# fxzjshm/simple-radio-telescope-backend

Hardware: AMD Instinct MI355X
Metric: baseband Msamples/sec/node + real-time ratio, J1644-4559 config at 1/2/4/8 MI355X (higher is better)
Workload: dtype fp32; 1 GPU; model=J1644-4559 coherent-dedispersion single-pulse pipeline, baseband_input_count=1073741824, nsamps_reserved=23494656, baseband_input_bits=2, spectrum_channel_count=2048, rfi=True, phase_table=False, fft_backend=native, parallelism=stream-sharded dp1, global_batch=1, seq_len=1073741824

## Files before the change

csrc/bind/module.cpp:

```cpp

#include <torch/extension.h>
#include <ATen/cuda/CUDAContext.h>
#include <c10/cuda/CUDAGuard.h>

#include <functional>
#include <vector>

#include "../engine/engine.h"
#include "../fft/native_fft.h"
#include "../include/srtb_kernels.h"

namespace {

using namespace srtb_hip;

hipStream_t cur_stream() {
  return at::cuda::getCurrentCUDAStream().stream();
}

void check(hipError_t e, const char* what) { check_hip(e, what); }

#define CHECK_CUDA(t) TORCH_CHECK((t).is_cuda(), #t " must be on GPU")
#define CHECK_CONTIG(t) TORCH_CHECK((t).is_contiguous(), #t " must be contiguous")

// ... 341 lines not shown
  CHECK_CONTIG(x);
  TORCH_CHECK(x.scalar_type() == torch::kComplexFloat);
  const size_t len = x.size(-1);
  const size_t batch = x.numel() / len;
  auto stream = cur_stream();
  NativeFft plan;
  plan.plan(len, batch, (int)sign, stream);
  auto out = torch::empty_like(x);
  if (plan.n_passes() == 1) {
    plan.exec(cptr(x), cptr(out), stream);
  } else {
    auto work = x.clone();
    plan.exec(cptr(work), cptr(out), stream);
  }
  check(hipStreamSynchronize(stream), "native_fft sync");
  return out;
}

torch::Tensor t_native_rfft(torch::Tensor x) {
  CHECK_CUDA(x);
  CHECK_CONTIG(x);
  TORCH_CHECK(x.scalar_type() == torch::kFloat32);
  const size_t n = x.numel();
  const size_t m = n / 2;
  auto stream = cur_stream();
  NativeFft plan;
  plan.plan(m, 1, -1, stream);
  auto z = torch::empty({(int64_t)m},
                        x.options().dtype(torch::kComplexFloat));
  auto packed = x.view({(int64_t)m, 2});
// ... 236 lines not shown
  m.def("sk_v1_mitigate", &t_sk_v1_mitigate, py::arg("wf"),
        py::arg("sk_threshold"), py::arg("normalize") = false);
  m.def("time_series", &t_time_series, py::arg("wf"), py::arg("flags"),
        py::arg("ts_count"));
  m.def("subtract_mean", &t_subtract_mean);
  m.def("count_signal", &t_count_signal);
  m.def("inclusive_scan", &t_inclusive_scan);
  m.def("boxcar", &t_boxcar);
  m.def("resample_power", &t_resample_power);
  m.def("normalize_by_mean", &t_normalize_by_mean);
  m.def("generate_pixmap", &t_generate_pixmap);
  m.def("running_mean", &t_running_mean);
  m.def("correlate", &t_correlate);
  m.def("native_fft", &t_native_fft, py::arg("x"), py::arg("sign"));
  m.def("native_rfft", &t_native_rfft, py::arg("x"));
  m.def("bench_fft", &t_bench_fft, py::arg("len"), py::arg("batch"),
        py::arg("sign"), py::arg("iters") = 20, py::arg("backend") = "native");
  m.def("bench_rfft", &t_bench_rfft, py::arg("n"), py::arg("iters") = 20,
        py::arg("backend") = "native");

  py::class_<PyEngine>(m, "PipelineEngine")
      .def(py::init<int64_t, int64_t, int64_t, double, double, double, double,
                    double, double, double, int64_t, int64_t,
                    std::vector<std::vector<int64_t>>, bool, bool, bool,
                    int64_t, int64_t, int64_t, bool>(),
           py::arg("n"), py::arg("nbits"), py::arg("channels"),
           py::arg("freq_low"), py::arg("bandwidth"), py::arg("sample_rate"),
           py::arg("dm"), py::arg("rfi_threshold") = 10.0,
           py::arg("sk_threshold") = 1.1, py::arg("snr_threshold") = 6.0,
           py::arg("max_boxcar") = 1024, py::arg("nsamps_reserved") = 0,
// ... 23 lines not shown
```

csrc/engine/engine.cpp:

```cpp
#include "engine.h"

#include <roctracer/roctx.h>

#include <cmath>
#include <cstdlib>
#include <cstring>
#include <stdexcept>

namespace srtb_hip {

namespace {
constexpr double kD = 4.148808e3;

struct RoctxRange {
  bool on;
  explicit RoctxRange(const char* name)
      : on([] {
          static const bool enabled = [] {
            const char* e = std::getenv("SRTB_ROCTX");
            return e && std::atoi(e) != 0;
          }();
          return enabled;
        }()) {
    if (on) roctxRangePush(name);
// ... 66 lines not shown
    if (n_boxcars_ > 0)
      check_hip(hipMalloc(&s.box_partials,
                          (size_t)n_boxcars_ * 2 * np * sizeof(double)),
                "box partials alloc");
    check_hip(hipMalloc(&s.mean_power, sizeof(double)), "mean alloc");
    check_hip(hipMalloc(&s.sums, 2 * sizeof(double)), "sums alloc");
    const int ncnt = 1 + 1 + n_boxcars_;
    check_hip(hipMalloc(&s.counters, ncnt * sizeof(unsigned)), "cnt alloc");
    check_hip(hipMalloc(&s.thresholds, (1 + n_boxcars_) * sizeof(float)),
              "thr alloc");
    check_hip(hipHostMalloc(&s.h_counters, ncnt * sizeof(unsigned)),
              "pinned cnt");
    check_hip(hipHostMalloc(&s.h_thresholds, (1 + n_boxcars_) * sizeof(float)),
              "pinned thr");
    fused_unpack_off_ = std::getenv("SRTB_NO_FUSED_UNPACK") != nullptr;
    const int be = cfg.fft_backend;
    native_fft_ = (be == 0 || be == 2) && NativeFft::supported(nc_);
    native_bwd_ = native_fft_ && NativeFft::supported(l_) &&
                  (be == 0 || l_ >= (1ull << 17));
    fuse_r2c_ = false;
    if (native_fft_) {
      s.nfwd.plan(nc_, 1, -1, s.stream);
      if (native_bwd_) {
        const char* b32 = std::getenv("SRTB_FFT_BWD32");
        if (b32 && std::atoi(b32) != 0)
          s.nbwd.plan(l_, s_, +1, s.stream, 5,
                      8);
        else
          s.nbwd.plan(l_, s_, +1, s.stream);
        const int wpr = s.nbwd.dif_sk_wgs_per_row();
// ... 78 lines not shown
  if (phase_table_) (void)hipFree(phase_table_);
  if (window_) (void)hipFree(window_);
  if (watfft_window_) (void)hipFree(watfft_window_);
}

void PipelineEngine::enqueue_chain(Slot& s, const uint8_t* dev_raw,
                                   const float* dev_samples, double dm,
                                   bool record_event) {
  hipStream_t st = s.stream;
  if (std::isnan(dm)) dm = cfg_.dm;
  const float2* table = phase_table_;
  if (table && dm != cfg_.dm)
    throw std::runtime_error("dm override requires use_phase_table=false");

  RoctxRange r_chain("srtb_block_chain");
  const float* fft_in = s.samples;
  const int in_bits = cfg_.baseband_input_bits;
  const bool fuse_unpack = dev_raw && native_fft_ && !fused_unpack_off_ &&
                           (in_bits == 1 || in_bits == 2 || in_bits == 4 ||
                            in_bits == 8 || in_bits == -8 ||
                            in_bits == 16 || in_bits == -16) &&
                           !window_ && slots_[0]->nfwd.first_pass_fusable();
  if (dev_raw && !fuse_unpack) {
    check_hip(unpack(dev_raw, s.samples, n_, cfg_.baseband_input_bits,
                     window_, st),
              "unpack");
  } else if (!dev_raw && native_fft_) {
    check_hip(hipMemcpyAsync(s.samples, dev_samples, n_ * sizeof(float),
                             hipMemcpyDeviceToDevice, st),
              "samples d2d");
  } else if (!dev_raw) {
    fft_in = dev_samples;
  }
  const bool fr2c = fuse_r2c_;
  if (native_fft_ && fr2c) {
    s.nfwd.exec(reinterpret_cast<float2*>(s.samples), s.spec, st,
                nullptr, cfg_.enable_rfi_s1 ? s.fwd_pw : nullptr,
                fuse_unpack ? dev_raw : nullptr, in_bits);
    if (cfg_.enable_rfi_s1)
      check_hip(r2c_mean_from_power(s.fwd_pw, fwd_pw_n_, s.spec, nc_,
                                    s.mean_power, st),
                "r2c mean");
  } else if (native_fft_) {
    s.nfwd.exec(reinterpret_cast<float2*>(s.samples), s.spec, st,
                nullptr, nullptr, fuse_unpack ? dev_raw : nullptr, in_bits);
    check_hip(r2c_post_process(
                  s.spec, s.spec, nc_,
                  cfg_.enable_rfi_s1 ? s.partials : nullptr,
                  cfg_.enable_rfi_s1 ? s.mean_power : nullptr, st),
              "r2c post");
  } else {
    s.plans.exec_r2c(const_cast<float*>(fft_in), s.spec);
    if (cfg_.enable_rfi_s1)
      check_hip(mean_power(s.spec, nc_, s.partials, s.mean_power, st),
                "meanp");
  }
  float2* wf;
  const bool fuse_into_bwd = native_bwd_ && s.nbwd.first_pass_fusable();
  if (fuse_into_bwd) {
    FftPreop pre;
    pre.mean_power = cfg_.enable_rfi_s1 ? s.mean_power : nullptr;
    pre.threshold = cfg_.rfi_threshold;
    pre.norm_coeff = norm_coeff_;
    pre.n_zap = cfg_.n_zap_ranges;
    for (int i = 0; i < cfg_.n_zap_ranges; ++i) pre.zap[i] = cfg_.zap_ranges[i];
    pre.f_min = f_min_;
    pre.f_c = f_c_;
    pre.df = df_;
    pre.dm = dm;
    pre.table = table;
    pre.r2c_m = fr2c ? nc_ : 0;
    s.nbwd.exec(s.spec, reinterpret_cast<float2*>(s.samples), st, &pre,
                watfft_window_ ? nullptr : s.sk_dif_partials, nullptr, 2,
                fr2c ? s.xbuf : nullptr);
    wf = reinterpret_cast<float2*>(s.samples);
  } else {
    check_hip(rfi_dedisperse_fused(
                  s.spec, nc_, cfg_.enable_rfi_s1 ? s.mean_power : nullptr,
                  cfg_.rfi_threshold, norm_coeff_, cfg_.zap_ranges,
                  cfg_.n_zap_ranges, f_min_, f_c_, df_, dm, table, st),
              "rfi+dedisp");
    if (native_bwd_) {
      s.nbwd.exec(s.spec, reinterpret_cast<float2*>(s.samples), st);
      wf = reinterpret_cast<float2*>(s.samples);
    } else {
      s.plans.exec_c2c_backward(s.spec);
// ... 37 lines not shown
    check_hip(boxcar_ladder(s.cumsum, ts_count_, boxcar_lengths_.data(),
                            n_boxcars_, s.box_partials, cfg_.snr_threshold,
                            s.thresholds + 1, s.counters + 2, st),
              "box ladder");
  }
  check_hip(hipMemcpyAsync(s.h_counters, s.counters, ncnt * sizeof(unsigned),
                           hipMemcpyDeviceToHost, st),
            "res d2h");
  check_hip(hipMemcpyAsync(s.h_thresholds, s.thresholds,
                           (1 + n_boxcars_) * sizeof(float),
                           hipMemcpyDeviceToHost, st),
            "thr d2h");
  if (record_event) {
    check_hip(hipEventRecord(s.done, st), "event record");
    s.busy = true;
  }
}

int PipelineEngine::submit(const void* host_bytes, size_t nbytes,
                           double dm_override) {
  if (nbytes != raw_bytes_) throw std::runtime_error("submit: wrong size");
  const int id = next_slot_;
  next_slot_ = (next_slot_ + 1) % n_slots_;
  Slot& s = *slots_[id];
  if (s.busy) {
    check_hip(hipEventSynchronize(s.done), "slot wait");
    s.busy = false;
  }
  const bool graph_ok = cfg_.use_hip_graph && std::isnan(dm_override);
  if (graph_ok && s.graph_exec && s.graph_host_src == host_bytes) {
// ... 118 lines not shown
```

csrc/engine/engine.h:

```cpp

#pragma once

#include <hip/hip_runtime.h>

#include <array>
#include <cstdint>
#include <memory>
#include <vector>

#include "../fft/fft_plans.h"
#include "../fft/native_fft.h"
#include "../include/srtb_kernels.h"

namespace srtb_hip {

struct EngineConfig {
  size_t baseband_input_count = 1ull << 28;
  int baseband_input_bits = 8;
  size_t spectrum_channel_count = 1ull << 15;
  double freq_low = 1000.0;
  double bandwidth = 500.0;
  double sample_rate = 1e9;
  double dm = 0.0;
  float rfi_threshold = 10.0f;
// ... 102 lines not shown
    double* box_partials = nullptr;
    double* mean_power = nullptr;
    double* sums = nullptr;
    unsigned* counters = nullptr;
    float* thresholds = nullptr;
    unsigned* h_counters = nullptr;
    float* h_thresholds = nullptr;
    FftPlanSet plans;
    NativeFft nfwd, nbwd;
    hipGraphExec_t graph_exec = nullptr;
    const void* graph_host_src = nullptr;
    int graph_pending = 0;
  };
  std::vector<std::unique_ptr<Slot>> slots_;
  int next_slot_ = 0;
};

}
```

csrc/fft/native_fft.h:

```cpp

#pragma once

#include <algorithm>
#include <cstdint>
#include <cstdlib>
#include <cmath>
#include <stdexcept>
#include <string>
#include <vector>

#include "../include/srtb_kernels.h"
#include "fft_plans.h"

namespace srtb_hip {

class NativeFft {
 public:
  static constexpr uint32_t kMaxPassLen = 4096;
  static int elems_per_wg() {
    const char* e = std::getenv("SRTB_FFT_ELEMS");
    int v = e ? std::atoi(e) : 4096;
    if (v < 512) v = 512;
    if (v > 8192) v = 8192;
    return v;
// ... 158 lines not shown
      p.dif.n_prefix = m - 1;
      for (int w = 0; w < m - 1; ++w) {
        p.dif.pf_bits[w] = ilog2z(f[w]);
        p.dif.pf_coef[w] = M[w + 1] / fn;
      }
      p.n_ffts = batch * (L / fn);
      p.tw_n = len_table(fn);
      passes_.push_back(p);
    }
  }

  int n_passes() const { return (int)passes_.size(); }

  bool first_pass_fusable() const {
    return !passes_.empty() && passes_[0].kind == PassKind::kCol;
  }

  int dif_sk_wgs_per_row() const {
    if (passes_.empty() || passes_.back().kind != PassKind::kDif) return 0;
    const Pass& p = passes_.back();
    const size_t per_row = (len_ / p.dif.n);
    const int F = dif_f(p);
    if (per_row % F != 0) return 0;
    return (int)(per_row / F);
  }

  void exec(const float2* in, float2* out, hipStream_t stream,
            const FftPreop* preop = nullptr,
            float2* dif_sk_partials = nullptr,
            const uint8_t* decode2_raw = nullptr, int decode_bits = 2,
// ... 174 lines not shown
```

csrc/include/srtb_kernels.h:

```cpp

#pragma once

#include <hip/hip_runtime.h>
#include <cstddef>
#include <cstdint>

namespace srtb_hip {

hipError_t unpack(const uint8_t* in, float* out, size_t out_count, int nbits,
                  const float* window, hipStream_t stream);

hipError_t unpack_interleaved_2pol(const int8_t* in, float* out0, float* out1,
                                   size_t count_per_pol, const float* window,
                                   hipStream_t stream);

hipError_t unpack_naocpsr_snap1(const int8_t* in, float* out0, float* out1,
                                size_t count_per_pol, const float* window,
                                hipStream_t stream);

hipError_t unpack_gznupsr_a1(const uint8_t* in, float* out0, float* out1,
                             float* out2, float* out3, int n_streams,
                             size_t count_per_stream, const float* window,
                             hipStream_t stream);

// ... 109 lines not shown
  double f_min = 0, f_c = 0, df = 0, dm = 0;
  const float2* table = nullptr;
  unsigned long long r2c_m = 0;
};

hipError_t r2c_mean_from_power(const float2* power_partials,
                               size_t n_partials, const float2* z0, size_t m,
                               double* out_mean, hipStream_t stream);

hipError_t fft_col_pass(const float2* in, float2* out, const FftPassDesc& d,
                        size_t n_ffts, int sign, const float2* tw_n,
                        const float2* tw_hi, const float2* tw_lo,
                        hipStream_t stream, const FftPreop* preop = nullptr,
                        const uint8_t* raw2 = nullptr, int raw_bits = 2);

struct DifFinalDesc {
  uint32_t n;
  unsigned long long out_c2;
  unsigned long long out_elem_coef;
  int n_prefix = 0;
  int pf_bits[4] = {0, 0, 0, 0};
  unsigned long long pf_coef[4] = {0, 0, 0, 0};
};
hipError_t fft_mid512_pass(const float2* in, float2* out,
                           const FftPassDesc& d, size_t n_ffts, int sign,
                           const float2* tw_n, hipStream_t stream);

hipError_t fft_dif_final(const float2* in, float2* out, const DifFinalDesc& d,
                         size_t n_ffts, int F, int sign, const float2* tw_n,
                         float2* sk_partials, hipStream_t stream);
// ... 35 lines not shown
```

csrc/kernels/common.h:

```cpp
#pragma once

#include <hip/hip_runtime.h>
#include <cstddef>
#include <cstdint>

namespace srtb_hip {

constexpr int kBlock = 256;
constexpr int kMaxBlocks = 4096;

inline dim3 grid_for(size_t n, int block = kBlock, int cap = kMaxBlocks) {
  size_t b = (n + block - 1) / block;
  if (b > static_cast<size_t>(cap)) b = cap;
  if (b == 0) b = 1;
  return dim3(static_cast<uint32_t>(b));
}

#define SRTB_CHECK_LAUNCH()                        \
  do {                                             \
    hipError_t err_ = hipGetLastError();           \
    if (err_ != hipSuccess) return err_;           \
  } while (0)


// ... 32 lines not shown

__device__ inline float2 srtb_dedisp_factor(size_t i, double f_min,
                                            double f_c, double df,
                                            double dm) {
  const double f = f_min + df * (double)i;
  const double r = (f - f_c) / f_c;
  const double k = (kDispersionConstantMHz * 1e6) * dm / f * (r * r);
  double k_int;
  const double k_frac = modf(k, &k_int);
  const float phi = (float)(-2.0 * M_PI * k_frac);
  float s, c;
  __sincosf(phi, &s, &c);
  return make_float2(c, s);
}

}
```

csrc/kernels/fft.hip:

```cpp

#include <cstdlib>
#include "common.h"
#include "../include/srtb_kernels.h"

namespace srtb_hip {

namespace {

__device__ inline float2 cmulf(float2 a, float2 b) {
  return make_float2(a.x * b.x - a.y * b.y, a.x * b.y + a.y * b.x);
}

}

struct FftPassDescDev {
  uint32_t n;
  int n_log2, f_log2;
  int d0_log2, d1_log2;
  unsigned long long in_c0, in_c1, in_c2;
  unsigned long long in_stride;
  unsigned long long out_c0, out_c1, out_c2;
  unsigned long long out_stride;
  unsigned long long tw_f0, tw_f1;
  unsigned long long tw_mask;
// ... 345 lines not shown
  if (k == 0) return make_float2(zk.x + zk.y, 0.0f);
  const float2 zm = zbase[m - k];
  const float2 zmc = make_float2(zm.x, -zm.y);
  const float2 even = make_float2(0.5f * (zk.x + zmc.x),
                                  0.5f * (zk.y + zmc.y));
  const float2 dif = make_float2(zk.x - zmc.x, zk.y - zmc.y);
  const float2 odd = make_float2(0.5f * dif.y, -0.5f * dif.x);
  const float phiw = (float)(-M_PI * (double)k / (double)m);
  float sw, cw;
  __sincosf(phiw, &sw, &cw);
  const float2 wo = make_float2(cw * odd.x - sw * odd.y,
                                cw * odd.y + sw * odd.x);
  return make_float2(even.x + wo.x, even.y + wo.y);
}

template <int N, bool TWIDDLE, int SIGN, bool PREOP, int DEC = 0>
__global__ void __launch_bounds__(256)
    k_fft_col(const float2* __restrict__ in, float2* __restrict__ out,
              FftPassDescDev d, unsigned long long n_ffts,
              const float2* __restrict__ tw_n,
              const float2* __restrict__ tw_hi,
              const float2* __restrict__ tw_lo, FftPreopDev pre,
              const uint8_t* __restrict__ raw2) {
  const unsigned long long id =
      (unsigned long long)xcd_swizzle(blockIdx.x, gridDim.x, d.tuning) *
          blockDim.x + threadIdx.x;
  if (id >= n_ffts) return;
  unsigned long long q0, q1, q2;
  digits(id, d, q0, q1, q2);
  const unsigned long long base = q0 * d.in_c0 + q1 * d.in_c1 + q2 * d.in_c2;
  float thr_mean = 0.f;
  if constexpr (PREOP) {
    if (pre.mean_power) thr_mean = pre.threshold * (float)(*pre.mean_power);
  }
  float2 v[N];
  const float2* __restrict__ colbase = in + base;
  const uint32_t stride32 = (uint32_t)d.in_stride;
#pragma unroll
  for (int i = 0; i < N; ++i) {
    const uint32_t off = (uint32_t)i * stride32;
    const unsigned long long flat = base + off;
    float2 x;
    if constexpr (DEC != 0) x = decN_load<DEC>(raw2, flat);
    else x = ld_stream(colbase + off, d.tuning);
    if constexpr (PREOP) {
      if (pre.r2c_m) x = r2c_combine_load(in, x, flat, pre.r2c_m);
      bool zap = pre.mean_power && (norm2(x) > thr_mean);
      for (int z = 0; z < pre.n_zap; ++z)
        zap |= (flat >= pre.zap[z].lo) & (flat <= pre.zap[z].hi);
      if (zap) {
        x = make_float2(0.f, 0.f);
      } else {
        if (pre.mean_power) {
          x.x *= pre.norm_coeff;
          x.y *= pre.norm_coeff;
        }
        x = cmulf(x, pre.table ? pre.table[flat]
                               : srtb_dedisp_factor(flat, pre.f_min, pre.f_c,
                                                    pre.df, pre.dm));
      }
    }
    v[col_sigma<N>(i)] = x;
  }
  col_fft<N, SIGN>(v, tw_n);
  float2* __restrict__ ocolbase = out + base;
#pragma unroll
  for (int k = 0; k < N; ++k) {
    float2 r = v[k];
    if constexpr (TWIDDLE) {
      const unsigned long long m_ =
          (q0 * d.tw_f0 * (unsigned long long)k) & d.tw_mask;
      r = cmulf(r, tw_eval(m_, d.tw_angle));
    }
    st_stream(ocolbase + (uint32_t)k * stride32, r, d.tuning);
  }
}


constexpr int col_sigma_inv64(int pos) {
  for (int i = 0; i < 64; ++i)
    if (col_sigma<64>(i) == pos) return i;
  return 0;
}

__device__ inline float2 shfl_xor1(float2 x) {
  return make_float2(__shfl_xor(x.x, 1, 64), __shfl_xor(x.y, 1, 64));
}

template <bool TWIDDLE, int SIGN, bool PREOP, int DEC = 0>
__global__ void __launch_bounds__(256)
    k_fft_col_pair64(const float2* __restrict__ in, float2* __restrict__ out,
                     FftPassDescDev d, unsigned long long n_ffts,
                     const float2* __restrict__ tw_n,
                     const float2* __restrict__ tw_hi,
                     const float2* __restrict__ tw_lo, FftPreopDev pre,
                     const uint8_t* __restrict__ raw2) {
  const unsigned long long tid =
      (unsigned long long)xcd_swizzle(blockIdx.x, gridDim.x, d.tuning) *
          blockDim.x + threadIdx.x;
  const unsigned long long id = tid >> 1;
  const int p = (int)(tid & 1);
  if (id >= n_ffts) return;
  unsigned long long q0, q1, q2;
  digits(id, d, q0, q1, q2);
  const unsigned long long base = q0 * d.in_c0 + q1 * d.in_c1 + q2 * d.in_c2;
  float thr_mean = 0.f;
  if constexpr (PREOP) {
    if (pre.mean_power) thr_mean = pre.threshold * (float)(*pre.mean_power);
  }
  float2 v[32];
  const float2* __restrict__ colbase = in + base;
  const uint32_t stride32 = (uint32_t)d.in_stride;
#pragma unroll
  for (int r = 0; r < 32; ++r) {
    const int i = p ? col_sigma_inv64(32 + r) : col_sigma_inv64(r);
    const uint32_t off = (uint32_t)i * stride32;
    float2 x;
    if constexpr (DEC != 0) x = decN_load<DEC>(raw2, base + off);
    else x = ld_stream(colbase + off, d.tuning);
    if constexpr (PREOP) {
      const unsigned long long flat = base + off;
      if (pre.r2c_m) x = r2c_combine_load(in, x, flat, pre.r2c_m);
      bool zap = pre.mean_power && (norm2(x) > thr_mean);
      for (int z = 0; z < pre.n_zap; ++z)
        zap |= (flat >= pre.zap[z].lo) & (flat <= pre.zap[z].hi);
      if (zap) {
        x = make_float2(0.f, 0.f);
      } else {
        if (pre.mean_power) {
          x.x *= pre.norm_coeff;
          x.y *= pre.norm_coeff;
        }
        x = cmulf(x, pre.table ? pre.table[flat]
                               : srtb_dedisp_factor(flat, pre.f_min, pre.f_c,
                                                    pre.df, pre.dm));
      }
    }
    v[r] = x;
  }
  col_stage<32, 4, 4, SIGN, 16>(v, tw_n);
  col_stage<32, 16, 4, SIGN, 4>(v, tw_n);
#pragma unroll
  for (int j = 0; j < 16; ++j) {
    const float2 ea = shfl_xor1(v[j]);
    const float2 eb = shfl_xor1(v[16 + j]);
    float2 a = p ? ea : v[j];
    float2 b = p ? eb : v[16 + j];
    float2 c = p ? v[j] : ea;
    float2 e = p ? v[16 + j] : eb;
    float2 w1, w2, w3;
// ... 17 lines not shown
      const unsigned long long m_ =
          (q0 * d.tw_f0 * (unsigned long long)k) & d.tw_mask;
      rr = cmulf(rr, tw_eval(m_, d.tw_angle));
    }
    st_stream(ocolbase + (uint32_t)k * stride32, rr, d.tuning);
  }
}


constexpr int col_sigma_inv32(int pos) {
  for (int i = 0; i < 32; ++i)
    if (col_sigma<32>(i) == pos) return i;
  return 0;
}

template <bool TWIDDLE, int SIGN, bool PREOP, int DEC = 0>
__global__ void __launch_bounds__(256)
    k_fft_col_pair32(const float2* __restrict__ in, float2* __restrict__ out,
                     FftPassDescDev d, unsigned long long n_ffts,
                     const float2* __restrict__ tw_n,
                     const float2* __restrict__ tw_hi,
                     const float2* __restrict__ tw_lo, FftPreopDev pre,
                     const uint8_t* __restrict__ raw2) {
  const unsigned long long tid =
      (unsigned long long)xcd_swizzle(blockIdx.x, gridDim.x, d.tuning) *
          blockDim.x + threadIdx.x;
  const unsigned long long id = tid >> 1;
  const int p = (int)(tid & 1);
  if (id >= n_ffts) return;
  unsigned long long q0, q1, q2;
  digits(id, d, q0, q1, q2);
  const unsigned long long base = q0 * d.in_c0 + q1 * d.in_c1 + q2 * d.in_c2;
  float thr_mean = 0.f;
  if constexpr (PREOP) {
    if (pre.mean_power) thr_mean = pre.threshold * (float)(*pre.mean_power);
  }
  float2 v[16];
  const float2* __restrict__ colbase = in + base;
  const uint32_t stride32 = (uint32_t)d.in_stride;
#pragma unroll
  for (int r = 0; r < 16; ++r) {
    const int i = p ? col_sigma_inv32(16 + r) : col_sigma_inv32(r);
    const uint32_t off = (uint32_t)i * stride32;
    float2 x;
    if constexpr (DEC != 0) x = decN_load<DEC>(raw2, base + off);
    else x = ld_stream(colbase + off, d.tuning);
    if constexpr (PREOP) {
      const unsigned long long flat = base + off;
      if (pre.r2c_m) x = r2c_combine_load(in, x, flat, pre.r2c_m);
      bool zap = pre.mean_power && (norm2(x) > thr_mean);
      for (int z = 0; z < pre.n_zap; ++z)
        zap |= (flat >= pre.zap[z].lo) & (flat <= pre.zap[z].hi);
      if (zap) {
        x = make_float2(0.f, 0.f);
      } else {
        if (pre.mean_power) {
          x.x *= pre.norm_coeff;
          x.y *= pre.norm_coeff;
        }
        x = cmulf(x, pre.table ? pre.table[flat]
                               : srtb_dedisp_factor(flat, pre.f_min, pre.f_c,
                                                    pre.df, pre.dm));
      }
    }
    v[r] = x;
  }
  col_stage<16, 4, 4, SIGN, 8>(v, tw_n);
  col_stage<16, 16, 4, SIGN, 2>(v, tw_n);
#pragma unroll
  for (int j = 0; j < 16; ++j) {
    const float2 other = shfl_xor1(v[j]);
    const float2 a = p ? other : v[j];
    const float2 b = p ? v[j] : other;
    const float2 w = (j == 0) ? make_float2(1.f, 0.f) : tw_n[j];
    const float2 y = cmulf(b, w);
    v[j] = p ? make_float2(a.x - y.x, a.y - y.y)
             : make_float2(a.x + y.x, a.y + y.y);
// ... 514 lines not shown
  } while (0)
  if (load_ffast) {
    if (store_ffast) DISPATCH2(true, true);
    else             DISPATCH2(true, false);
  } else {
    if (store_ffast) DISPATCH2(false, true);
    else             DISPATCH2(false, false);
  }
#undef DISPATCH2
#undef DISPATCH4
  SRTB_CHECK_LAUNCH();
  return hipSuccess;
}


hipError_t fft_col_pass(const float2* in, float2* out, const FftPassDesc& hd,
                        size_t n_ffts, int sign, const float2* tw_n,
                        const float2* tw_hi, const float2* tw_lo,
                        hipStream_t stream, const FftPreop* preop,
                        const uint8_t* raw2, int raw_bits) {
  if (raw2 && (preop || hd.tw_mod == 0)) return hipErrorInvalidValue;
  if (raw2 && raw_bits != 1 && raw_bits != 2 && raw_bits != 4 &&
      raw_bits != 8 && raw_bits != -8 && raw_bits != 16 && raw_bits != -16)
    return hipErrorInvalidValue;
  FftPreopDev pre{};
  if (preop) {
    pre.mean_power = preop->mean_power;
    pre.threshold = preop->threshold;
    pre.norm_coeff = preop->norm_coeff;
    pre.n_zap = preop->n_zap;
    for (int i = 0; i < preop->n_zap; ++i) pre.zap[i] = preop->zap[i];
    pre.f_min = preop->f_min;
    pre.f_c = preop->f_c;
    pre.df = preop->df;
    pre.dm = preop->dm;
    pre.table = preop->table;
    pre.r2c_m = preop->r2c_m;
  }
  FftPassDescDev d;
  d.n = hd.n;
  d.n_log2 = ilog2(hd.n);
  d.f_log2 = 0;
  d.d0_log2 = hd.d0 ? ilog2(hd.d0) : 48;
  d.d1_log2 = ilog2(hd.d1 ? hd.d1 : 1);
  d.in_c0 = hd.in_c0; d.in_c1 = hd.in_c1; d.in_c2 = hd.in_c2;
  d.in_stride = hd.in_stride;
  d.out_c0 = hd.out_c0; d.out_c1 = hd.out_c1; d.out_c2 = hd.out_c2;
  d.out_stride = hd.out_stride;
  d.tw_f0 = hd.tw_f0; d.tw_f1 = hd.tw_f1;
  d.tw_mask = hd.tw_mod ? hd.tw_mod - 1 : 0;
  d.tw_lo_bits = hd.tw_lo_bits;
  d.tw_angle = hd.tw_angle;
  d.tuning = fft_tuning();
// ... 11 lines not shown
#define COL_DISPATCH_D(N)                                                    \
  if (raw_bits == 1) { if (sign < 0) COL_LAUNCH_D(N, -1, 1);                 \
                       else COL_LAUNCH_D(N, 1, 1); }                         \
  else if (raw_bits == 2) { if (sign < 0) COL_LAUNCH_D(N, -1, 2);            \
                            else COL_LAUNCH_D(N, 1, 2); }                    \
  else if (raw_bits == 4) { if (sign < 0) COL_LAUNCH_D(N, -1, 4);            \
                            else COL_LAUNCH_D(N, 1, 4); }                    \
  else if (raw_bits == 8) { if (sign < 0) COL_LAUNCH_D(N, -1, 8);            \
                            else COL_LAUNCH_D(N, 1, 8); }                    \
  else if (raw_bits == -8) { if (sign < 0) COL_LAUNCH_D(N, -1, -8);          \
                             else COL_LAUNCH_D(N, 1, -8); }                  \
  else if (raw_bits == 16) { if (sign < 0) COL_LAUNCH_D(N, -1, 16);          \
                             else COL_LAUNCH_D(N, 1, 16); }                  \
  else { if (sign < 0) COL_LAUNCH_D(N, -1, -16);                             \
         else COL_LAUNCH_D(N, 1, -16); }
#define COL_DISPATCH(N)                                                      \
  case N:                                                                    \
    if (raw2) {                                                              \
      COL_DISPATCH_D(N)                                                      \
    } else if (twiddle) {                                                           \
      if (sign < 0) { if (preop) COL_LAUNCH(N, true, -1, true);              \
                      else COL_LAUNCH(N, true, -1, false); }                 \
      else          { if (preop) COL_LAUNCH(N, true, 1, true);               \
                      else COL_LAUNCH(N, true, 1, false); }                  \
    } else {                                                                 \
      if (sign < 0) { if (preop) COL_LAUNCH(N, false, -1, true);             \
                      else COL_LAUNCH(N, false, -1, false); }                \
      else          { if (preop) COL_LAUNCH(N, false, 1, true);              \
                      else COL_LAUNCH(N, false, 1, false); }                 \
    }                                                                        \
    break;
  const uint32_t grid2 = (uint32_t)((2 * n_ffts + 255) / 256);
#define COL_LAUNCH_P(TW, SG, PR)                                             \
// ... 6 lines not shown
                     tw_lo, pre, raw2)
#define COL_LAUNCH_P32(TW, SG, PR)                                           \
  hipLaunchKernelGGL((k_fft_col_pair32<TW, SG, PR>), dim3(grid2), dim3(256), \
                     0, stream, in, out, d, n_ffts, tw_n, tw_hi, tw_lo, pre, \
                     raw2)
#define COL_LAUNCH_P32D(SG, B)                                               \
  hipLaunchKernelGGL((k_fft_col_pair32<true, SG, false, B>), dim3(grid2),    \
                     dim3(256), 0, stream, in, out, d, n_ffts, tw_n, tw_hi,  \
                     tw_lo, pre, raw2)
  switch (hd.n) {
    COL_DISPATCH(2)
    COL_DISPATCH(4)
    COL_DISPATCH(8)
    COL_DISPATCH(16)
    case 32:
      if (use_pair32()) {
        if (raw2) {
          if (raw_bits == 1) { if (sign < 0) COL_LAUNCH_P32D(-1, 1);
                               else COL_LAUNCH_P32D(1, 1); }
          else if (raw_bits == 2) { if (sign < 0) COL_LAUNCH_P32D(-1, 2);
                                    else COL_LAUNCH_P32D(1, 2); }
          else if (raw_bits == 4) { if (sign < 0) COL_LAUNCH_P32D(-1, 4);
                                    else COL_LAUNCH_P32D(1, 4); }
          else if (raw_bits == 8) { if (sign < 0) COL_LAUNCH_P32D(-1, 8);
                                    else COL_LAUNCH_P32D(1, 8); }
          else if (raw_bits == -8) { if (sign < 0) COL_LAUNCH_P32D(-1, -8);
                                     else COL_LAUNCH_P32D(1, -8); }
          else if (raw_bits == 16) { if (sign < 0) COL_LAUNCH_P32D(-1, 16);
                                     else COL_LAUNCH_P32D(1, 16); }
          else { if (sign < 0) COL_LAUNCH_P32D(-1, -16);
// ... 18 lines not shown
        break;
      }
      if (twiddle) {
        if (sign < 0) { if (preop) COL_LAUNCH(32, true, -1, true);
                        else COL_LAUNCH(32, true, -1, false); }
        else          { if (preop) COL_LAUNCH(32, true, 1, true);
                        else COL_LAUNCH(32, true, 1, false); }
      } else {
        if (sign < 0) { if (preop) COL_LAUNCH(32, false, -1, true);
                        else COL_LAUNCH(32, false, -1, false); }
        else          { if (preop) COL_LAUNCH(32, false, 1, true);
                        else COL_LAUNCH(32, false, 1, false); }
      }
      break;
    case 64:
      if (raw2) {
        if (raw_bits == 1) { if (sign < 0) COL_LAUNCH_PD(-1, 1);
                             else COL_LAUNCH_PD(1, 1); }
        else if (raw_bits == 2) { if (sign < 0) COL_LAUNCH_PD(-1, 2);
                                  else COL_LAUNCH_PD(1, 2); }
        else if (raw_bits == 4) { if (sign < 0) COL_LAUNCH_PD(-1, 4);
                                  else COL_LAUNCH_PD(1, 4); }
        else if (raw_bits == 8) { if (sign < 0) COL_LAUNCH_PD(-1, 8);
                                  else COL_LAUNCH_PD(1, 8); }
        else if (raw_bits == -8) { if (sign < 0) COL_LAUNCH_PD(-1, -8);
                                   else COL_LAUNCH_PD(1, -8); }
        else if (raw_bits == 16) { if (sign < 0) COL_LAUNCH_PD(-1, 16);
                                   else COL_LAUNCH_PD(1, 16); }
        else { if (sign < 0) COL_LAUNCH_PD(-1, -16);
               else COL_LAUNCH_PD(1, -16); }
// ... 6 lines not shown
                        else COL_LAUNCH_P(true, 1, false); }
      } else {
        if (sign < 0) { if (preop) COL_LAUNCH_P(false, -1, true);
                        else COL_LAUNCH_P(false, -1, false); }
        else          { if (preop) COL_LAUNCH_P(false, 1, true);
                        else COL_LAUNCH_P(false, 1, false); }
      }
      break;
    default:
      return hipErrorInvalidValue;
  }
#undef COL_DISPATCH
#undef COL_DISPATCH_D
#undef COL_LAUNCH
#undef COL_LAUNCH_D
#undef COL_LAUNCH_P
#undef COL_LAUNCH_PD
#undef COL_LAUNCH_P32
#undef COL_LAUNCH_P32D
  SRTB_CHECK_LAUNCH();
  return hipSuccess;
}

hipError_t fft_mid512_pass(const float2* in, float2* out,
                           const FftPassDesc& hd, size_t n_ffts, int sign,
                           const float2* tw_n, hipStream_t stream) {
  if (hd.n != 512 || hd.tw_mod == 0) return hipErrorInvalidValue;
  FftPassDescDev d;
  d.n = hd.n;
  d.n_log2 = 9;
// ... 184 lines not shown
```

Before: 62830 Msamples/s.

## Evaluate dedispersion chirp via fixed-point cubic polynomial per FFT column

Adds a POLY variant of the backward FFT column kernels. Each column sets up a cubic phase polynomial in 64-bit fixed-point turns once, then evaluates it per element with integer multiply-adds and hardware sin/cos, replacing the per-element double-precision dedispersion phase. Zap ranges become a precomputed bitmask. The path is enabled only when an error bound on the dropped higher-order terms is small, and it also adds optional chain serialization across slots plus test bindings. The trade-off is a small phase approximation error and possible loss of cross-slot overlap, since by default chains are ordered whenever the poly path is used.

Result: faster. 66040 Msamples/s, median of 6 (+5.1%).

```diff
diff --git a/csrc/bind/module.cpp b/csrc/bind/module.cpp
--- a/csrc/bind/module.cpp
+++ b/csrc/bind/module.cpp
@@ -379,6 +379,65 @@
     plan.exec(cptr(work), cptr(out), stream);
   }
   check(hipStreamSynchronize(stream), "native_fft sync");
+  return out;
+}
+
+std::tuple<std::vector<torch::Tensor>, std::vector<bool>> t_preop_backward_fft(
+    torch::Tensor spec, int64_t maxcol_log2, int64_t final_log2, double f_min,
+    double f_c, double df, std::vector<double> dms,
+    std::vector<std::vector<int64_t>> ranges, bool enable_rfi,
+    double threshold, int64_t channel_count) {
+  CHECK_CUDA(spec);
+  CHECK_CONTIG(spec);
+  TORCH_CHECK(spec.scalar_type() == torch::kComplexFloat);
+  TORCH_CHECK(ranges.size() <= 16, "at most 16 zap ranges");
+  const size_t len = spec.size(-1);
+  const size_t n = spec.numel();
+  const size_t batch = n / len;
+  auto stream = cur_stream();
+  NativeFft plan;
+  plan.plan(len, batch, +1, stream, (int)maxcol_log2, (int)final_log2);
+  TORCH_CHECK(plan.first_pass_fusable(), "plan has no column first pass");
+  torch::Tensor mean;
+  FftPreop pre;
+  if (enable_rfi) {
+    mean = t_mean_power(spec);
+    pre.mean_power = mean.data_ptr<double>();
+    pre.threshold = (float)threshold;
+    pre.norm_coeff =
+        (float)std::pow((double)n * (double)n / (double)channel_count, -0.5);
+  }
+  pre.n_zap = (int)ranges.size();
+  for (size_t i = 0; i < ranges.size(); ++i) {
+    pre.zap[i].lo = (unsigned long long)ranges[i][0];
+    pre.zap[i].hi = (unsigned long long)ranges[i][1];
+  }
+  pre.f_min = f_min;
+  pre.f_c = f_c;
+  pre.df = df;
+  std::vector<torch::Tensor> outs;
+  std::vector<bool> poly;
+  for (double dm : dms) {
+    pre.dm = dm;
+    poly.push_back(plan.preop_uses_poly(pre));
+    auto work = spec.clone();
+    auto out = torch::empty_like(spec);
+    plan.exec(cptr(work), cptr(out), stream, &pre);
+    outs.push_back(out);
+  }
+  check(hipStreamSynchronize(stream), "preop_backward_fft sync");
+  return {outs, poly};
+}
+
+torch::Tensor t_dedisp_poly_factors(int64_t nc, int64_t n, int64_t stride,
+                                    double f_min, double f_c, double df,
+                                    double dm, torch::Device dev) {
+  auto out = torch::empty({nc}, torch::TensorOptions()
+                                    .dtype(torch::kComplexFloat)
+                                    .device(dev));
+  check(dedisp_poly_factors(cptr(out), (size_t)nc, (uint32_t)n,
+                            (size_t)stride, f_min, f_c, df, dm, cur_stream()),
+        "dedisp_poly_factors");
   return out;
 }
 
@@ -645,6 +704,13 @@
   m.def("correlate", &t_correlate);
   m.def("native_fft", &t_native_fft, py::arg("x"), py::arg("sign"));
   m.def("native_rfft", &t_native_rfft, py::arg("x"));
+  m.def("preop_backward_fft", &t_preop_backward_fft, py::arg("spec"),
+        py::arg("maxcol_log2"), py::arg("final_log2"), py::arg("f_min"),
+        py::arg("f_c"), py::arg("df"), py::arg("dms"),
+        py::arg("ranges") = std::vector<std::vector<int64_t>>{},
+        py::arg("enable_rfi") = false, py::arg("threshold") = 0.0,
+        py::arg("channel_count") = 1);
+  m.def("dedisp_poly_factors", &t_dedisp_poly_factors);
   m.def("bench_fft", &t_bench_fft, py::arg("len"), py::arg("batch"),
         py::arg("sign"), py::arg("iters") = 20, py::arg("backend") = "native");
   m.def("bench_rfft", &t_bench_rfft, py::arg("n"), py::arg("iters") = 20,
diff --git a/csrc/engine/engine.cpp b/csrc/engine/engine.cpp
--- a/csrc/engine/engine.cpp
+++ b/csrc/engine/engine.cpp
@@ -104,6 +104,8 @@
     check_hip(hipHostMalloc(&s.h_thresholds, (1 + n_boxcars_) * sizeof(float)),
               "pinned thr");
     fused_unpack_off_ = std::getenv("SRTB_NO_FUSED_UNPACK") != nullptr;
+    if (const char* sc = std::getenv("SRTB_SERIAL_CHAINS"))
+      serial_chains_ = std::atoi(sc) != 0 ? 1 : 0;
     const int be = cfg.fft_backend;
     native_fft_ = (be == 0 || be == 2) && NativeFft::supported(nc_);
     native_bwd_ = native_fft_ && NativeFft::supported(l_) &&
@@ -212,6 +214,26 @@
     throw std::runtime_error("dm override requires use_phase_table=false");
 
   RoctxRange r_chain("srtb_block_chain");
+  const bool fr2c = fuse_r2c_;
+  const bool fuse_into_bwd = native_bwd_ && s.nbwd.first_pass_fusable();
+  FftPreop pre;
+  if (fuse_into_bwd) {
+    pre.mean_power = cfg_.enable_rfi_s1 ? s.mean_power : nullptr;
+    pre.threshold = cfg_.rfi_threshold;
+    pre.norm_coeff = norm_coeff_;
+    pre.n_zap = cfg_.n_zap_ranges;
+    for (int i = 0; i < cfg_.n_zap_ranges; ++i) pre.zap[i] = cfg_.zap_ranges[i];
+    pre.f_min = f_min_;
+    pre.f_c = f_c_;
+    pre.df = df_;
+    pre.dm = dm;
+    pre.table = table;
+    pre.r2c_m = fr2c ? nc_ : 0;
+  }
+  if (record_event && last_chain_done_ && last_chain_done_ != s.done &&
+      (serial_chains_ > 0 ||
+       (serial_chains_ < 0 && fuse_into_bwd && s.nbwd.preop_uses_poly(pre))))
+    check_hip(hipStreamWaitEvent(st, last_chain_done_, 0), "chain order");
   const float* fft_in = s.samples;
   const int in_bits = cfg_.baseband_input_bits;
   const bool fuse_unpack = dev_raw && native_fft_ && !fused_unpack_off_ &&
@@ -230,7 +252,6 @@
   } else if (!dev_raw) {
     fft_in = dev_samples;
   }
-  const bool fr2c = fuse_r2c_;
   if (native_fft_ && fr2c) {
     s.nfwd.exec(reinterpret_cast<float2*>(s.samples), s.spec, st,
                 nullptr, cfg_.enable_rfi_s1 ? s.fwd_pw : nullptr,
@@ -254,20 +275,7 @@
                 "meanp");
   }
   float2* wf;
-  const bool fuse_into_bwd = native_bwd_ && s.nbwd.first_pass_fusable();
   if (fuse_into_bwd) {
-    FftPreop pre;
-    pre.mean_power = cfg_.enable_rfi_s1 ? s.mean_power : nullptr;
-    pre.threshold = cfg_.rfi_threshold;
-    pre.norm_coeff = norm_coeff_;
-    pre.n_zap = cfg_.n_zap_ranges;
-    for (int i = 0; i < cfg_.n_zap_ranges; ++i) pre.zap[i] = cfg_.zap_ranges[i];
-    pre.f_min = f_min_;
-    pre.f_c = f_c_;
-    pre.df = df_;
-    pre.dm = dm;
-    pre.table = table;
-    pre.r2c_m = fr2c ? nc_ : 0;
     s.nbwd.exec(s.spec, reinterpret_cast<float2*>(s.samples), st, &pre,
                 watfft_window_ ? nullptr : s.sk_dif_partials, nullptr, 2,
                 fr2c ? s.xbuf : nullptr);
@@ -335,6 +343,7 @@
   if (record_event) {
     check_hip(hipEventRecord(s.done, st), "event record");
     s.busy = true;
+    last_chain_done_ = s.done;
   }
 }
 
diff --git a/csrc/engine/engine.h b/csrc/engine/engine.h
--- a/csrc/engine/engine.h
+++ b/csrc/engine/engine.h
@@ -140,6 +140,8 @@
   };
   std::vector<std::unique_ptr<Slot>> slots_;
   int next_slot_ = 0;
+  hipEvent_t last_chain_done_ = nullptr;
+  int serial_chains_ = -1;
 };
 
 }
diff --git a/csrc/fft/native_fft.h b/csrc/fft/native_fft.h
--- a/csrc/fft/native_fft.h
+++ b/csrc/fft/native_fft.h
@@ -196,6 +196,12 @@
 
   bool first_pass_fusable() const {
     return !passes_.empty() && passes_[0].kind == PassKind::kCol;
+  }
+
+  bool preop_uses_poly(const FftPreop& preop) const {
+    return first_pass_fusable() &&
+           fft_col_preop_uses_poly(passes_[0].d, passes_[0].n_ffts, sign_,
+                                   preop);
   }
 
   int dif_sk_wgs_per_row() const {
diff --git a/csrc/include/srtb_kernels.h b/csrc/include/srtb_kernels.h
--- a/csrc/include/srtb_kernels.h
+++ b/csrc/include/srtb_kernels.h
@@ -147,6 +147,13 @@
                         hipStream_t stream, const FftPreop* preop = nullptr,
                         const uint8_t* raw2 = nullptr, int raw_bits = 2);
 
+bool fft_col_preop_uses_poly(const FftPassDesc& d, size_t n_ffts, int sign,
+                             const FftPreop& preop);
+
+hipError_t dedisp_poly_factors(float2* out, size_t nc, uint32_t n,
+                               size_t stride, double f_min, double f_c,
+                               double df, double dm, hipStream_t stream);
+
 struct DifFinalDesc {
   uint32_t n;
   unsigned long long out_c2;
diff --git a/csrc/kernels/common.h b/csrc/kernels/common.h
--- a/csrc/kernels/common.h
+++ b/csrc/kernels/common.h
@@ -70,4 +70,38 @@
   return make_float2(c, s);
 }
 
+struct DedispPoly {
+  unsigned long long c0, c1, c2, c3;
+};
+
+__device__ inline unsigned long long srtb_turns_to_fix64(double t) {
+  const double fr = t - floor(t);
+  return fr < 1.0 ? (unsigned long long)(fr * 18446744073709551616.0) : 0ull;
 }
+
+__device__ inline DedispPoly srtb_dedisp_poly_setup(unsigned long long bin0,
+                                                    unsigned long long stride,
+                                                    double f_min, double f_c,
+                                                    double df, double dm) {
+  const double f0 = f_min + df * (double)bin0;
+  const double r = (f0 - f_c) / f_c;
+  const double q = (kDispersionConstantMHz * 1e6) * dm / f0;
+  const double u = df * (double)stride / f0;
+  DedispPoly p;
+  p.c0 = srtb_turns_to_fix64(q * (r * r));
+  p.c1 = srtb_turns_to_fix64(q * r * (r + 2.0) * u);
+  p.c2 = srtb_turns_to_fix64(q * (u * u));
+  p.c3 = srtb_turns_to_fix64(-q * (u * u) * u);
+  return p;
+}
+
+__device__ __forceinline__ float2 srtb_dedisp_poly_eval(const DedispPoly& p,
+                                                        unsigned j) {
+  const unsigned long long jj = j;
+  const unsigned long long t = p.c0 + jj * (p.c1 + jj * (p.c2 + jj * p.c3));
+  const float turns = (float)(int)(unsigned)(t >> 32) * 0x1p-32f;
+  return make_float2(__builtin_amdgcn_cosf(turns),
+                     -__builtin_amdgcn_sinf(turns));
+}
+
+}
diff --git a/csrc/kernels/fft.hip b/csrc/kernels/fft.hip
--- a/csrc/kernels/fft.hip
+++ b/csrc/kernels/fft.hip
@@ -1,4 +1,5 @@
 
+#include <cmath>
 #include <cstdlib>
 #include "common.h"
 #include "../include/srtb_kernels.h"
@@ -383,7 +384,56 @@
   return make_float2(even.x + wo.x, even.y + wo.y);
 }
 
-template <int N, bool TWIDDLE, int SIGN, bool PREOP, int DEC = 0>
+__device__ __forceinline__ float2 preop_apply(const float2* __restrict__ in,
+                                              float2 x,
+                                              unsigned long long flat,
+                                              const FftPreopDev& pre,
+                                              float thr_mean) {
+  if (pre.r2c_m) x = r2c_combine_load(in, x, flat, pre.r2c_m);
+  bool zap = pre.mean_power && (norm2(x) > thr_mean);
+  for (int z = 0; z < pre.n_zap; ++z)
+    zap |= (flat >= pre.zap[z].lo) & (flat <= pre.zap[z].hi);
+  if (zap) return make_float2(0.f, 0.f);
+  if (pre.mean_power) {
+    x.x *= pre.norm_coeff;
+    x.y *= pre.norm_coeff;
+  }
+  return cmulf(x, pre.table ? pre.table[flat]
+                            : srtb_dedisp_factor(flat, pre.f_min, pre.f_c,
+                                                 pre.df, pre.dm));
+}
+
+template <int R, typename FlatFn>
+__device__ __forceinline__ uint32_t preop_zap_mask(const FftPreopDev& pre,
+                                                   unsigned long long first,
+                                                   unsigned long long last,
+                                                   FlatFn flat_of) {
+  static_assert(R <= 32, "one mask bit per register element");
+  uint32_t mask = 0;
+  for (int z = 0; z < pre.n_zap; ++z) {
+    const unsigned long long lo = pre.zap[z].lo, hi = pre.zap[z].hi;
+    if (hi < first || lo > last) continue;
+#pragma unroll
+    for (int r = 0; r < R; ++r) {
+      const unsigned long long flat = flat_of(r);
+      mask |= (uint32_t)((flat >= lo) & (flat <= hi)) << r;
+    }
+  }
+  return mask;
+}
+
+__device__ __forceinline__ float2 preop_poly_apply(float2 x, bool zap_bit,
+                                                   float thr, float nc,
+                                                   const DedispPoly& poly,
+                                                   unsigned j) {
+  const bool zap = zap_bit | (norm2(x) > thr);
+  const float2 y = cmulf(make_float2(x.x * nc, x.y * nc),
+                         srtb_dedisp_poly_eval(poly, j));
+  return zap ? make_float2(0.f, 0.f) : y;
+}
+
+template <int N, bool TWIDDLE, int SIGN, bool PREOP, int DEC = 0,
+          bool POLY = false>
 __global__ void __launch_bounds__(256)
     k_fft_col(const float2* __restrict__ in, float2* __restrict__ out,
               FftPassDescDev d, unsigned long long n_ffts,
@@ -399,8 +449,20 @@
   digits(id, d, q0, q1, q2);
   const unsigned long long base = q0 * d.in_c0 + q1 * d.in_c1 + q2 * d.in_c2;
   float thr_mean = 0.f;
+  [[maybe_unused]] float norm_c = 1.f;
+  [[maybe_unused]] DedispPoly poly{};
+  [[maybe_unused]] uint32_t zap_mask = 0;
   if constexpr (PREOP) {
     if (pre.mean_power) thr_mean = pre.threshold * (float)(*pre.mean_power);
+    if constexpr (POLY) {
+      if (pre.mean_power) norm_c = pre.norm_coeff;
+      else thr_mean = __builtin_inff();
+      poly = srtb_dedisp_poly_setup(base, d.in_stride, pre.f_min, pre.f_c,
+                                    pre.df, pre.dm);
+      zap_mask = preop_zap_mask<N>(
+          pre, base, base + (N - 1) * d.in_stride,
+          [&](int i) { return base + (unsigned)i * d.in_stride; });
+    }
   }
   float2 v[N];
   const float2* __restrict__ colbase = in + base;
@@ -413,20 +475,11 @@
     if constexpr (DEC != 0) x = decN_load<DEC>(raw2, flat);
     else x = ld_stream(colbase + off, d.tuning);
     if constexpr (PREOP) {
-      if (pre.r2c_m) x = r2c_combine_load(in, x, flat, pre.r2c_m);
-      bool zap = pre.mean_power && (norm2(x) > thr_mean);
-      for (int z = 0; z < pre.n_zap; ++z)
-        zap |= (flat >= pre.zap[z].lo) & (flat <= pre.zap[z].hi);
-      if (zap) {
-        x = make_float2(0.f, 0.f);
+      if constexpr (POLY) {
+        x = preop_poly_apply(x, (zap_mask >> i) & 1u, thr_mean, norm_c, poly,
+                             i);
       } else {
-        if (pre.mean_power) {
-          x.x *= pre.norm_coeff;
-          x.y *= pre.norm_coeff;
-        }
-        x = cmulf(x, pre.table ? pre.table[flat]
-                               : srtb_dedisp_factor(flat, pre.f_min, pre.f_c,
-                                                    pre.df, pre.dm));
+        x = preop_apply(in, x, flat, pre, thr_mean);
       }
     }
     v[col_sigma<N>(i)] = x;
@@ -456,7 +509,8 @@
   return make_float2(__shfl_xor(x.x, 1, 64), __shfl_xor(x.y, 1, 64));
 }
 
-template <bool TWIDDLE, int SIGN, bool PREOP, int DEC = 0>
+template <bool TWIDDLE, int SIGN, bool PREOP, int DEC = 0,
+          bool POLY = false>
 __global__ void __launch_bounds__(256)
     k_fft_col_pair64(const float2* __restrict__ in, float2* __restrict__ out,
                      FftPassDescDev d, unsigned long long n_ffts,
@@ -474,8 +528,22 @@
   digits(id, d, q0, q1, q2);
   const unsigned long long base = q0 * d.in_c0 + q1 * d.in_c1 + q2 * d.in_c2;
   float thr_mean = 0.f;
+  [[maybe_unused]] float norm_c = 1.f;
+  [[maybe_unused]] DedispPoly poly{};
+  [[maybe_unused]] uint32_t zap_mask = 0;
   if constexpr (PREOP) {
     if (pre.mean_power) thr_mean = pre.threshold * (float)(*pre.mean_power);
+    if constexpr (POLY) {
+      if (pre.mean_power) norm_c = pre.norm_coeff;
+      else thr_mean = __builtin_inff();
+      const unsigned long long first = base + 2ull * p * d.in_stride;
+      poly = srtb_dedisp_poly_setup(first, d.in_stride, pre.f_min, pre.f_c,
+                                    pre.df, pre.dm);
+      zap_mask = preop_zap_mask<32>(
+          pre, first, first + 61 * d.in_stride, [&](int r) {
+            return first + (unsigned)col_sigma_inv64(r) * d.in_stride;
+          });
+    }
   }
   float2 v[32];
   const float2* __restrict__ colbase = in + base;
@@ -489,20 +557,11 @@
     else x = ld_stream(colbase + off, d.tuning);
     if constexpr (PREOP) {
       const unsigned long long flat = base + off;
-      if (pre.r2c_m) x = r2c_combine_load(in, x, flat, pre.r2c_m);
-      bool zap = pre.mean_power && (norm2(x) > thr_mean);
-      for (int z = 0; z < pre.n_zap; ++z)
-        zap |= (flat >= pre.zap[z].lo) & (flat <= pre.zap[z].hi);
-      if (zap) {
-        x = make_float2(0.f, 0.f);
+      if constexpr (POLY) {
+        x = preop_poly_apply(x, (zap_mask >> r) & 1u, thr_mean, norm_c, poly,
+                             col_sigma_inv64(r));
       } else {
-        if (pre.mean_power) {
-          x.x *= pre.norm_coeff;
-          x.y *= pre.norm_coeff;
-        }
-        x = cmulf(x, pre.table ? pre.table[flat]
-                               : srtb_dedisp_factor(flat, pre.f_min, pre.f_c,
-                                                    pre.df, pre.dm));
+        x = preop_apply(in, x, flat, pre, thr_mean);
       }
     }
     v[r] = x;
@@ -550,7 +609,8 @@
   return 0;
 }
 
-template <bool TWIDDLE, int SIGN, bool PREOP, int DEC = 0>
+template <bool TWIDDLE, int SIGN, bool PREOP, int DEC = 0,
+          bool POLY = false>
 __global__ void __launch_bounds__(256)
     k_fft_col_pair32(const float2* __restrict__ in, float2* __restrict__ out,
                      FftPassDescDev d, unsigned long long n_ffts,
@@ -568,8 +628,22 @@
   digits(id, d, q0, q1, q2);
   const unsigned long long base = q0 * d.in_c0 + q1 * d.in_c1 + q2 * d.in_c2;
   float thr_mean = 0.f;
+  [[maybe_unused]] float norm_c = 1.f;
+  [[maybe_unused]] DedispPoly poly{};
+  [[maybe_unused]] uint32_t zap_mask = 0;
   if constexpr (PREOP) {
     if (pre.mean_power) thr_mean = pre.threshold * (float)(*pre.mean_power);
+    if constexpr (POLY) {
+      if (pre.mean_power) norm_c = pre.norm_coeff;
+      else thr_mean = __builtin_inff();
+      const unsigned long long first = base + 1ull * p * d.in_stride;
+      poly = srtb_dedisp_poly_setup(first, d.in_stride, pre.f_min, pre.f_c,
+                                    pre.df, pre.dm);
+      zap_mask = preop_zap_mask<16>(
+          pre, first, first + 30 * d.in_stride, [&](int r) {
+            return first + (unsigned)col_sigma_inv32(r) * d.in_stride;
+          });
+    }
   }
   float2 v[16];
   const float2* __restrict__ colbase = in + base;
@@ -583,20 +657,11 @@
     else x = ld_stream(colbase + off, d.tuning);
     if constexpr (PREOP) {
       const unsigned long long flat = base + off;
-      if (pre.r2c_m) x = r2c_combine_load(in, x, flat, pre.r2c_m);
-      bool zap = pre.mean_power && (norm2(x) > thr_mean);
-      for (int z = 0; z < pre.n_zap; ++z)
-        zap |= (flat >= pre.zap[z].lo) & (flat <= pre.zap[z].hi);
-      if (zap) {
-        x = make_float2(0.f, 0.f);
+      if constexpr (POLY) {
+        x = preop_poly_apply(x, (zap_mask >> r) & 1u, thr_mean, norm_c, poly,
+                             col_sigma_inv32(r));
       } else {
-        if (pre.mean_power) {
-          x.x *= pre.norm_coeff;
-          x.y *= pre.norm_coeff;
-        }
-        x = cmulf(x, pre.table ? pre.table[flat]
-                               : srtb_dedisp_factor(flat, pre.f_min, pre.f_c,
-                                                    pre.df, pre.dm));
+        x = preop_apply(in, x, flat, pre, thr_mean);
       }
     }
     v[r] = x;
@@ -1141,6 +1206,74 @@
 }
 
 
+static bool dedisp_poly_enabled() {
+  const char* e = std::getenv("SRTB_DEDISP_POLY");
+  return e ? (std::atoi(e) != 0) : true;
+}
+
+bool fft_col_preop_uses_poly(const FftPassDesc& hd, size_t n_ffts, int sign,
+                             const FftPreop& preop) {
+  if (!dedisp_poly_enabled()) return false;
+  if (preop.table || preop.r2c_m) return false;
+  if (sign <= 0 || hd.tw_mod == 0) return false;
+  if (hd.n < 2 || hd.n > 64) return false;
+  const double f_a = preop.f_min;
+  const double f_b =
+      preop.f_min + preop.df * (double)(n_ffts * (size_t)hd.n - 1);
+  if (!(f_a * f_b > 0.0)) return false;
+  const double f_lo = std::fmin(std::fabs(f_a), std::fabs(f_b));
+  const double span =
+      std::fabs(preop.df) * (double)hd.in_stride * (double)(hd.n - 1);
+  const double x = span / f_lo;
+  const double bound =
+      std::fabs(kDispersionConstantMHz * 1e6 * preop.dm) / f_lo * (x * x) *
+      (x * x);
+  return bound <= 0x1p-28;
+}
+
+namespace {
+template <int N>
+__global__ void k_dedisp_poly_factors(float2* __restrict__ out,
+                                      unsigned long long n_cols,
+                                      unsigned long long stride, double f_min,
+                                      double f_c, double df, double dm) {
+  const unsigned long long id =
+      (unsigned long long)blockIdx.x * blockDim.x + threadIdx.x;
+  if (id >= n_cols) return;
+  const unsigned long long base = (id / stride) * (N * stride) + id % stride;
+  const DedispPoly poly =
+      srtb_dedisp_poly_setup(base, stride, f_min, f_c, df, dm);
+#pragma unroll
+  for (int j = 0; j < N; ++j)
+    out[base + (unsigned long long)j * stride] =
+        srtb_dedisp_poly_eval(poly, j);
+}
+}
+
+hipError_t dedisp_poly_factors(float2* out, size_t nc, uint32_t n,
+                               size_t stride, double f_min, double f_c,
+                               double df, double dm, hipStream_t stream) {
+  if (stride == 0 || nc == 0 || nc % ((size_t)n * stride) != 0)
+    return hipErrorInvalidValue;
+  const size_t n_cols = nc / n;
+  const dim3 grid((uint32_t)((n_cols + 255) / 256));
+#define POLYF_CASE(NN)                                                       \
+  case NN:                                                                   \
+    hipLaunchKernelGGL((k_dedisp_poly_factors<NN>), grid, dim3(256), 0,      \
+                       stream, out, (unsigned long long)n_cols,              \
+                       (unsigned long long)stride, f_min, f_c, df, dm);      \
+    break;
+  switch (n) {
+    POLYF_CASE(2) POLYF_CASE(4) POLYF_CASE(8) POLYF_CASE(16) POLYF_CASE(32)
+    POLYF_CASE(64)
+    default:
+      return hipErrorInvalidValue;
+  }
+#undef POLYF_CASE
+  SRTB_CHECK_LAUNCH();
+  return hipSuccess;
+}
+
 hipError_t fft_col_pass(const float2* in, float2* out, const FftPassDesc& hd,
                         size_t n_ffts, int sign, const float2* tw_n,
                         const float2* tw_hi, const float2* tw_lo,
@@ -1164,6 +1297,8 @@
     pre.table = preop->table;
     pre.r2c_m = preop->r2c_m;
   }
+  const bool poly =
+      preop && !raw2 && fft_col_preop_uses_poly(hd, n_ffts, sign, *preop);
   FftPassDescDev d;
   d.n = hd.n;
   d.n_log2 = ilog2(hd.n);
@@ -1205,9 +1340,15 @@
                              else COL_LAUNCH_D(N, 1, 16); }                  \
   else { if (sign < 0) COL_LAUNCH_D(N, -1, -16);                             \
          else COL_LAUNCH_D(N, 1, -16); }
+#define COL_LAUNCH_POLY(N)                                                   \
+  hipLaunchKernelGGL((k_fft_col<N, true, 1, true, 0, true>), dim3(grid),     \
+                     dim3(256), 0, stream, in, out, d, n_ffts, tw_n, tw_hi,  \
+                     tw_lo, pre, raw2)
 #define COL_DISPATCH(N)                                                      \
   case N:                                                                    \
-    if (raw2) {                                                              \
+    if (poly) {                                                              \
+      COL_LAUNCH_POLY(N);                                                    \
+    } else if (raw2) {                                                       \
       COL_DISPATCH_D(N)                                                      \
     } else if (twiddle) {                                                           \
       if (sign < 0) { if (preop) COL_LAUNCH(N, true, -1, true);              \
@@ -1244,6 +1385,15 @@
     COL_DISPATCH(8)
     COL_DISPATCH(16)
     case 32:
+      if (poly) {
+        if (use_pair32())
+          hipLaunchKernelGGL((k_fft_col_pair32<true, 1, true, 0, true>),
+                             dim3(grid2), dim3(256), 0, stream, in, out, d,
+                             n_ffts, tw_n, tw_hi, tw_lo, pre, raw2);
+        else
+          COL_LAUNCH_POLY(32);
+        break;
+      }
       if (use_pair32()) {
         if (raw2) {
           if (raw_bits == 1) { if (sign < 0) COL_LAUNCH_P32D(-1, 1);
@@ -1292,6 +1442,12 @@
       }
       break;
     case 64:
+      if (poly) {
+        hipLaunchKernelGGL((k_fft_col_pair64<true, 1, true, 0, true>),
+                           dim3(grid2), dim3(256), 0, stream, in, out, d,
+                           n_ffts, tw_n, tw_hi, tw_lo, pre, raw2);
+        break;
+      }
       if (raw2) {
         if (raw_bits == 1) { if (sign < 0) COL_LAUNCH_PD(-1, 1);
                              else COL_LAUNCH_PD(1, 1); }
@@ -1328,6 +1484,7 @@
 #undef COL_DISPATCH_D
 #undef COL_LAUNCH
 #undef COL_LAUNCH_D
+#undef COL_LAUNCH_POLY
 #undef COL_LAUNCH_P
 #undef COL_LAUNCH_PD
 #undef COL_LAUNCH_P32
```
